# JuliaRobotics/KernelDensityEstimate.jl

Measured on AMD Instinct MI355X. Metric: gibbs_product_samples_per_sec, higher is better.
Workload: dtype f64

## Files before the change

kerneldensityestimate.jl_amd/csrc/gibbs_device.hpp:

```cpp
#pragma once
#include <hip/hip_runtime.h>

#include <cstdint>
#include <type_traits>

#include "circ_wrap.hpp"
#include "fastexp.hpp"
#include "kdehip_internal.hpp"
#include "philox.hpp"


namespace kdehip {


__device__ __forceinline__ double fast_rcp(double x) {
  double r = __builtin_amdgcn_rcp(x);
  double e = fma(-x, r, 1.0);
  r = fma(r, e, r);
  e = fma(-x, r, 1.0);
  return fma(r, e, r);
}
__device__ __forceinline__ float fast_rcp(float x) {
  float r = __builtin_amdgcn_rcpf(x);
  return fmaf(r, fmaf(-x, r, 1.0f), r);
// ... 765 lines not shown
template <int WAVES>
__device__ __forceinline__ void stage_tile(const unsigned char *__restrict__ src, unsigned char *dst,
                                           int bytes, int wave, int lane) {
  const __amdgpu_buffer_rsrc_t rsrc =
      __builtin_amdgcn_make_buffer_rsrc(const_cast<unsigned char *>(src), 0, bytes, 0x00020000);
  const int pieces = bytes >> 10;
  for (int c = wave; c < pieces; c += WAVES) {
    const int off = __builtin_amdgcn_readfirstlane(c << 10);
    __builtin_amdgcn_raw_ptr_buffer_load_lds(rsrc, (LdsVoidPtr)(dst + off), 16, lane << 4, off, 0, 0);
  }
}

template <bool BATCH>
struct LaunchView {
  const PlanDev &plan;
  const RunArgs &a;
  unsigned block;
  __device__ __forceinline__ LaunchView(const PlanDev &p, const RunArgs &a_) : plan(p), a(a_), block(blockIdx.x) {}
};
struct BatchArgs {
  int64_t Np;
  int32_t Niter, addEntropy, variant, use_tables;
  static constexpr int32_t use_screen = 0;
  uint64_t seed;
  int64_t sample_offset;
  double *points;
  int64_t *indices;
  int32_t *labels;
  static constexpr int32_t rng_philox = 1, npeers = 0, table_build = 0;
  static constexpr const double *randU = nullptr, *randN = nullptr;
  static constexpr int64_t K = 0, R = 0, nU = 0, nN = 0;
  double *peer_points[1];
  int64_t *peer_indices[1];
};
template <>
struct LaunchView<true> {
  PlanDev plan;
  BatchArgs a;
  unsigned block;
  __device__ __forceinline__ LaunchView(const PlanDev &, const RunArgs &a_) {
    const int e = ((const __attribute__((address_space(4))) int *)(a_.batch_map))[blockIdx.x];
    const auto *src = (const __attribute__((address_space(4))) kdehip_v16i *)(a_.batch + e);
    const kdehip_v16i r0 = src[0], r1 = src[1], r2 = src[2];
    BatchPlanHead h;
    BatchRun be;
    BatchFlags fl;
    __builtin_memcpy(&h, &r0, sizeof(h));
    __builtin_memcpy(&be, &r1, sizeof(be));
    __builtin_memcpy(&fl, &r2, sizeof(fl));
    plan.data = h.data; plan.perm = h.perm; plan.levels = h.levels; plan.tables = h.tables; plan.tabdesc = h.tabdesc;
    plan.tab_rows_total = h.tab_rows_total;
    plan.M = h.M; plan.L = h.L; plan.D = h.D; plan.Lt = h.Lt;
    plan.screened = 0;
    plan.circ_bits = fl.circ_bits;
    a.Np = be.Np; a.Niter = fl.Niter; a.addEntropy = fl.addEntropy; a.use_tables = fl.use_tables;
    a.variant = a_.variant;
    a.seed = be.seed; a.sample_offset = be.sample_offset;
    a.points = be.points; a.indices = be.indices; a.labels = be.labels;
    a.peer_points[0] = nullptr; a.peer_indices[0] = nullptr;
    block = blockIdx.x - static_cast<unsigned>(fl.first_block);
  }
};


}
```

kerneldensityestimate.jl_amd/csrc/gibbs_lean.hip:

```cpp
#define KDEHIP_EXP256 1
#ifndef KDEHIP_PRELOAD_MAXB
#define KDEHIP_PRELOAD_MAXB 8
#endif
#include "gibbs_device.hpp"
#include "screen_device.hpp"

namespace kdehip {

template <int I> using IC = std::integral_constant<int, I>;
template <int N, int I = 0, typename F>
__device__ __forceinline__ void static_for(F &&f) {
  if constexpr (I < N) {
    f(IC<I>{});
    static_for<N, I + 1>(f);
  }
}

#if defined(KDEHIP_LEAN_HI) || (defined(KDEHIP_LEAN_DEV_M) && KDEHIP_LEAN_DEV_M > 4)
constexpr int kLeanMinDens = 8, kLeanMaxDens = 8;
#else
constexpr int kLeanMinDens = 2, kLeanMaxDens = 4;
#endif
constexpr int kLeanMaxNormals = 128;

__device__ __forceinline__ int scalar_copy(int x) {
  int y;
  asm("s_mov_b32 %0, %1" : "=s"(y) : "s"(x));
  return y;
}

template <int D>
struct LeanTile {
  int n;
  int flags;
  int lds_off;
  int stage_bytes;
  int chunk_rows;
  int seg;
  int hdr_lo, hdr_hi;
  int B, F, last_lane;
  int uniform_bw;
  __device__ __forceinline__ int64_t hdr_off() const {
    return (static_cast<int64_t>(hdr_hi) << 32) | static_cast<uint32_t>(hdr_lo);
  }
  __device__ __forceinline__ void load(const kdehip_v8i &d) {
    n = scalar_copy(d[0]);
    flags = scalar_copy(d[1]);
    lds_off = scalar_copy(d[2]);
    stage_bytes = scalar_copy(d[3]);
    chunk_rows = scalar_copy(d[4]);
    seg = scalar_copy(d[5]);
    hdr_lo = scalar_copy(d[6]);
    hdr_hi = scalar_copy(d[7]);
    B = (n + 63) >> 6;
    last_lane = flags & 0xFF;
    uniform_bw = flags >> 8;
    F = uniform_bw ? D + 1 : 2 * D + 1;
  }
};

template <typename P, typename T, bool OK> constexpr bool kCanPreloadImpl = OK && kIsLdsPtr<P> && sizeof(T) == 8;

template <typename T, int D, int M, int WAVES, bool BATCH = false, bool SCHUNK = false>
__global__ __launch_bounds__(WAVES * 64) void gibbs_lean_kernel(PlanDev plan_, RunArgs a_) {
  const LaunchView<BATCH> view(plan_, a_);
  const PlanDev &plan = view.plan;
  const auto &a = view.a;
  constexpr bool kPrefetchRows = (WAVES <= 12) || sizeof(T) == 4 || D <= 4;
  using RowPtr = std::conditional_t<(WAVES == 16 && sizeof(T) == 8), LdsPtrSplit<T>, LdsPtr<T>>;
  constexpr int kCopyWaves = WAVES > 4 ? 4 : WAVES;
  constexpr bool kKeptRows = (WAVES <= 8);
  constexpr bool kScreen = sizeof(T) == 8 && !BATCH;
  constexpr bool kPreloadBuild = kKeptRows && kPrefetchRows;
  constexpr int kNormOff = 2048;
  constexpr int kUnifOff = kNormOff + WAVES * kLeanMaxNormals * 8;
  constexpr int kPoolOff = kUnifOff + WAVES * 1024;
  constexpr bool kCoop = kScreen && SCHUNK && WAVES == 8;
  constexpr int kXchgOff = kPoolOff + kLdsPoolBytes;
  constexpr int kXchgSlotDoubles = 32 + 4 * 64;
  constexpr int kXchgBytes = kCoop ? 64 + WAVES * kXchgSlotDoubles * 8 : 0;
  static_assert(kPoolOff + kLdsPoolBytes + kXchgBytes <= 160 * 1024, "LDS budget of one CU exceeded");
  __shared__ __attribute__((aligned(1024))) unsigned char smem[kPoolOff + kLdsPoolBytes + kXchgBytes];

  double *sExpTab = reinterpret_cast<double *>(smem);
  if (threadIdx.x < 256) sExpTab[threadIdx.x] = kExp2Tab256[threadIdx.x];
  if constexpr (kCoop) {
    if (threadIdx.x < 16) reinterpret_cast<int *>(smem + kXchgOff)[threadIdx.x] = 0;
  }

  const int lane = threadIdx.x & 63;
  const int wave = __builtin_amdgcn_readfirstlane(static_cast<int>(threadIdx.x >> 6));
  KDEHIP_PRIO_CHAIN();
  const int chain = wave;
  int64_t s = static_cast<int64_t>(view.block) * WAVES + chain;
  const bool live = s < a.Np;
  if (!live) s = a.Np - 1;
  const uint64_t gs = static_cast<uint64_t>(a.sample_offset + s);
  const void *fb = live ? static_cast<const void *>(plan.levels) : nullptr;

  const int L = plan.L;
  const T *__restrict__ data = static_cast<const T *>(plan.data);
  const LevelTable levels{(const __attribute__((address_space(4))) kdehip_v16i *)(plan.levels)};
  const StepTable steps{(const __attribute__((address_space(4))) kdehip_v8i *)(plan.levels + 2 * plan.M * (plan.L + 1))};
  unsigned char *pool = smem + kPoolOff;
  const int dl = lane < D ? lane : D - 1;
  const int vlev = a.variant % 1000;

  double *sNorm = reinterpret_cast<double *>(smem + kNormOff) + chain * kLeanMaxNormals;
  const int R = D * (L + 1);
  if (a.rng_philox) {
    for (int b = lane; 2 * b < R; b += 64) {
      double n0, n1;
      philox_normal_pair(a.seed, gs, static_cast<uint32_t>(b), n0, n1);
      sNorm[2 * b] = n0;
      if (2 * b + 1 < R) sNorm[2 * b + 1] = n1;
    }
  } else {
    for (int r = lane; r < R; r += 64) sNorm[r] = a.randN[s * a.R + r];
  }
  __syncthreads();

  T lam[M], lmu[M];
  int psel[M];

  auto adopt = [&](auto jc, const auto &ds, auto hdr, int pos) {
    constexpr int j = decltype(jc)::value;
    using TA = TileAddr<T>;
    auto e = hdr + kTileHeader + TA::row(pos >> 6, TA::stride(ds.F)) + (pos & 63) * TA::kLane;
    const T mu = e[dl * TA::kField];
    const T var = ds.uniform_bw ? hdr[dl] : e[(D + dl) * TA::kField];
    const T l = fast_rcp(var);
    lam[j] = l;
    lmu[j] = mu * l;
    psel[j] = pos;
  };
  auto product = [&](auto skipc, T &mean, T &cov) {
    constexpr int skip = decltype(skipc)::value;
    T ls = T(0), ms = T(0);
    static_for<M>([&](auto kc) {
      constexpr int k = decltype(kc)::value;
      if constexpr (k != skip) { ls += lam[k]; ms += lmu[k]; }
    });
    cov = fast_rcp(ls);
    mean = cov * ms;
  };

  auto draw = [&](const auto &ds, auto hdr, T mean, T cov, auto &&run) -> int {
    if (ds.uniform_bw) {
      EvalUniform<T, D> ev;
      ev.tab = sExpTab;
      const T c = hdr[dl] + cov;
      T cen, nin;
      EvalUniform<T, D>::operands(mean, c, true, cen, nin);
      T Pr = T(1);
#pragma unroll
      for (int d = 0; d < D; ++d) {
        ev.center[d] = lane_read(cen, d);
        ev.ninv[d] = lane_read(nin, d);
        Pr *= lane_read(c, d);
      }
      ev.scale = Num<T>::rsqrt(Pr);
      return run(ev);
    }
    EvalFast<T, D, false> ev;
    ev.tab = sExpTab;
    ev.act = 0;
#pragma unroll
    for (int d = 0; d < D; ++d) {
      ev.center[d] = lane_read(mean, d);
      ev.cov[d] = lane_read(cov, d);
    }
    return run(ev);
  };

  uint32_t c = static_cast<uint32_t>(M);
  uint32_t ubatch = 0xFFFFFFFFu;
  double *sUnif = reinterpret_cast<double *>(smem + kUnifOff) + wave * 128;
  auto next_uniform = [&]() -> double {
    const uint32_t b = c >> 7;
    if (b != ubatch) {
      ubatch = b;
      double u_even, u_odd;
      if (a.rng_philox) {
        const Philox4 r = philox_block(a.seed, gs, b * 64u + static_cast<uint32_t>(lane), 0u);
        u_even = bits_to_unit(r.v[0], r.v[1]);
        u_odd = bits_to_unit(r.v[2], r.v[3]);
      } else {
        const int64_t i0 = s * a.K + static_cast<int64_t>(b) * 128 + 2 * lane - 1;
        u_even = (i0 >= 0 && i0 < a.nU) ? a.randU[i0] : 0.5;
        u_odd = (i0 + 1 < a.nU) ? a.randU[i0 + 1] : 0.5;
      }
      wave_sync();
      sUnif[2 * lane] = u_even;
      sUnif[2 * lane + 1] = u_odd;
      wave_sync();
    }
    const double u = sUnif[c & 127u];
    ++c;
    return u;
  };

  static_for<M>([&](auto jc) {
    const LevelDesc ds = levels[decltype(jc)::value * (L + 1)];
    adopt(jc, ds, data + ds.hdr_off, 0);
  });

  const TabTable tabs{(const __attribute__((address_space(4))) kdehip_v8i *)(plan.tabdesc)};
  const T *tables = static_cast<const T *>(plan.tables);
  const int Lt = (vlev == 1 || vlev == 4 || !a.use_tables) ? 0 : plan.Lt;

  auto draw_rows = [&](const auto &ds, auto rows, const auto &ev, double u) -> int {
    using P = decltype(rows);
    return draw_label<T, P, kPrefetchRows, kKeptRows>(rows, ds, lane, ev, u, fb);
  };

  auto draw_rows_repeat = [&](const auto &ds, const T *rows, const auto &ev, double u) -> int {
    using Ev = std::decay_t<decltype(ev)>;
    if constexpr (kScreen && SCHUNK && sizeof(typename Ev::Row) <= 7 * sizeof(T) && WAVES <= 8) {
      LaneAcc<T> acc;
      KDEHIP_PRIO_ROWS();
      lane_rows_all_deep<T, Ev>(rows, ds.B, TileAddr<T>::stride(ds.F), lane, ev, acc);
      KDEHIP_PRIO_CHAIN();
      return select_or_raise<T, const T *>(acc.total(), rows, ds, lane, ev, u, fb);
    }
    return draw_rows(ds, rows, ev, u);
  };

#ifdef KDEHIP_SCREEN_STAMPS
  unsigned long long rstamp[8] = {0, 0, 0, 0, 0, 0, 0, 0}, r_prev_end = 0;
  bool rstamp_on = false;
#define RSTAMP(var) const unsigned long long var = __builtin_amdgcn_s_memtime()
#define RSTAMP_ADD(slot, t0, t1) do { if (rstamp_on) rstamp[slot] += (t1) - (t0); } while (0)
#else
#define RSTAMP(var) do {} while (0)
#define RSTAMP_ADD(slot, t0, t1) do {} while (0)
#endif
  auto step_kept = [&](auto jc, const auto &ds, auto hdr, const auto &row, T mean, T cov, double u) {
    RSTAMP(tr1);
    auto rows1 = hdr + kTileHeader;
    using P1 = decltype(rows1);
    using Ev = EvalFast<T, D, false>;
    Ev ev;
    ev.tab = sExpTab;
    ev.act = 0;
#pragma unroll
    for (int d = 0; d < D; ++d) {
      ev.center[d] = lane_read(mean, d);
      ev.cov[d] = lane_read(cov, d);
    }
#ifdef KDEHIP_SCREEN_STAMPS
    asm volatile("" ::"s"(ev.center[D - 1]), "s"(ev.cov[D - 1]));
#endif
    RSTAMP(tr2);
    RSTAMP_ADD(1, tr1, tr2);
    int pos1;
    if (ds.B == 1) {
      const T S = ev(row);
      pos1 = select_or_raise<T, P1>(S, rows1, ds, lane, ev, u, fb);
    } else if (ds.B <= 4) {
      pos1 = draw_label_kept<T, P1, Ev, 4>(rows1, ds, lane, ev, u, fb, row);
    } else {
// ... 212 lines not shown
          ev.scale = __builtin_amdgcn_rsqf(pr);
          pos = screen_draw<D, true>(rows32, ds.n, ds.B, ds.F, lane, ev, u SSTAMP_ARGS);
        } else {
          ScreenEval<D, false> ev;
          ev.a2 = a2; ev.nsum = (ds.B + 1) >> 1; ev.scale = 1.0f;
#pragma unroll
          for (int d = 0; d < D; ++d) {
            ev.cen[d] = lane_read(cen, d);
            ev.b[d] = lane_read(covf, d);
          }
          pos = screen_draw<D, false>(rows32, ds.n, ds.B, ds.F, lane, ev, u SSTAMP_ARGS);
        }
        pos = __builtin_amdgcn_readfirstlane(pos);
      }
      SSTAMP(ts2);
      SSTAMP_ADD(1, ts1, ts2);
      ++n_screened;
      if (pos < 0) {
        ++n_repeated;
        pos = __builtin_amdgcn_readfirstlane(draw(ds, hdrg, mean, cov, [&](const auto &ev) {
          return draw_rows_repeat(ds, hdrg + kTileHeader, ev, u);
        }));
      }
      SSTAMP(ts3);
      SSTAMP_ADD(2, ts2, ts3);
      adopt(jc, ds, hdrg, pos);
#ifdef KDEHIP_SCREEN_STAMPS
      {
        const double sink = lam[decltype(jc)::value] + lmu[decltype(jc)::value];
        asm volatile("" ::"v"(sink));
      }
#endif
      SSTAMP(ts4);
      SSTAMP_ADD(3, ts3, ts4);
    }
  };

  int gchunk = 0;
  auto stage_chunk = [&](const auto &ds, int r0, int half) {
    using TA = TileAddr<T>;
    const int RS = TA::stride(ds.F), rc = ds.chunk_rows;
    const int nrows = (ds.B - r0 < rc) ? (ds.B - r0) : rc;
    const int bytes = (static_cast<int>(TA::span(nrows, RS)) * int(sizeof(T)) + 1023) & ~1023;
    const unsigned char *src = reinterpret_cast<const unsigned char *>(data + ds.hdr_off() + kTileHeader + TA::row(r0, RS));
    if (wave < kCopyWaves) stage_tile<kCopyWaves>(src, pool + half * (kLdsPoolBytes / 2), bytes, wave, lane);
  };

  auto stage_schunk = [&](const LevelDesc &sc, int p0, int half) {
    using TA = TileAddr<float>;
    const int RS = TA::stride(sc.F), cp = sc.chunk_rows >> 1, npairs = (sc.B + 1) >> 1;
    const int np = (npairs - p0 < cp) ? (npairs - p0) : cp;
    const int head = p0 == 0 ? kScreenHeaderFloats : 0;
    const int bytes = ((head + np * RS) * 4 + 1023) & ~1023;
    const unsigned char *src = reinterpret_cast<const unsigned char *>(reinterpret_cast<const float *>(plan.data) + sc.hdr_off +
                                                                       (p0 == 0 ? 0 : kScreenHeaderFloats + p0 * RS));
    if (wave < kCopyWaves) stage_tile<kCopyWaves>(src, pool + half * (kLdsPoolBytes / 2), bytes, wave, lane);
  };
  auto step_screen_chunked = [&](auto jc, const auto &ds, const auto &dsp, const LevelDesc &sc, const LevelDesc &scn, bool more,
                                 bool first, bool level_start, T x) {
    if constexpr (kScreen && SCHUNK) {
      using TA = TileAddr<float>;
      T mean = x, cov = T(0);
      const bool was_pend = kCoop && pend;
      if (!first && !was_pend) product(jc, mean, cov);
      const double u = next_uniform();
      const int RS = TA::stride(sc.F), cp = sc.chunk_rows >> 1, npairs = (sc.B + 1) >> 1;
      staging_barrier();
      if (cp < npairs) stage_schunk(sc, cp, (gchunk + 1) & 1);
      else if (more) stage_schunk(scn, 0, (gchunk + 1) & 1);
      if constexpr (kCoop) {
        constexpr int j = decltype(jc)::value;
        if (!level_start) coop_resolve(IC<(j + M - 1) % M>{}, dsp, (cstep + 1) & 1);
        if (was_pend && !first) product(jc, mean, cov);
      }
      const LdsPtr<float> h32 = (LdsPtr<float>)(pool + (gchunk & 1) * (kLdsPoolBytes / 2));
      const LdsPtr<double> h64 = (LdsPtr<double>)(pool + (gchunk & 1) * (kLdsPoolBytes / 2));
      const double mu0 = h64[dl], cmin = h64[8 + dl];
      const float mmax = h32[32 + dl], valid = h32[40];
      const float *grows = reinterpret_cast<const float *>(plan.data) + sc.hdr_off + kScreenHeaderFloats;
      const int pos = __builtin_amdgcn_readfirstlane(screen_eval(ds, mu0, cmin, mmax, valid, mean, cov, [&](const auto &ev, bool ok) {
        using Ev = std::decay_t<decltype(ev)>;
        ScreenSums q;
        KDEHIP_PRIO_ROWS();
        if (ok) screen_rows<D, Ev::kUni>(h32 + kScreenHeaderFloats + lane * TA::kLane, npairs < cp ? npairs : cp, RS, ev, q);
        ++gchunk;
        for (int p0 = cp; p0 < npairs; p0 += cp, ++gchunk) {
          staging_barrier();
          if (p0 + cp < npairs) stage_schunk(sc, p0 + cp, (gchunk + 1) & 1);
          else if (more) stage_schunk(scn, 0, (gchunk + 1) & 1);
          const int np = (npairs - p0 < cp) ? (npairs - p0) : cp;
          if (ok) screen_rows<D, Ev::kUni>((LdsPtr<float>)(pool + (gchunk & 1) * (kLdsPoolBytes / 2)) + lane * TA::kLane, np, RS, ev, q);
        }
        KDEHIP_PRIO_CHAIN();
        if (!ok) return -1;
        return screen_decide<D, Ev::kUni, true>(grows, ds.n, ds.B, RS, lane, ev, u, q.values(), q.moments() SSTAMP_ARGS);
      }));
      if constexpr (kCoop) {
        ++n_screened;
        if (pos < 0) {
          ++n_repeated;
          coop_post(mean, cov, u);
        } else {
          adopt(jc, ds, data + ds.hdr_off(), pos);
        }
        ++cstep;
      } else {
        screen_finish(jc, ds, pos, mean, cov, u);
      }
    }
  };

#ifdef KDEHIP_EXPERIMENTS
  const int Lrun = (vlev >= 100 && vlev - 100 < L) ? vlev - 100 : L;
#else
  const int Lrun = L;
#endif
  for (int l = 1; l <= Lrun; ++l) {
    T x;
    {
      T mean, cov;
      product(IC<-1>{}, mean, cov);
      x = mean + Num<T>::sqrt(cov) * static_cast<T>(sNorm[(l - 1) * D + dl]);
    }
    const int level_mode = scalar_copy(levels[l].stage_mode);
    auto tile_raw = [&](int j) -> kdehip_v8i { return steps.raw(j * (L + 1) + l); };
    auto tile = [&](int j) -> LeanTile<D> {
      LeanTile<D> t;
      t.load(tile_raw(j));
      return t;
    };
    const int mode = vlev == 1 ? int(kStageGlobal) : level_mode;
    const bool tabulated = (l <= Lt);
    const int npass = tabulated ? 1 : a.Niter + 1;

    bool screened = false, screen_streamed = false, screen_chunked = false;
    if constexpr (kScreen) {
      if (a.use_screen && vlev != 1) {
        const int smode = scalar_copy(levels[M * (L + 1) + l].stage_mode);
        screened = smode == kStageScreen;
        screen_streamed = smode == kStageScreenStream;
        if constexpr (SCHUNK) screen_chunked = smode == kStageScreenChunked;
      }
    }
#ifdef KDEHIP_SCREEN_STAMPS
    rstamp_on = (vlev >= 300 && l == vlev - 300) && view.block == 3 && wave == 5;
    r_prev_end = 0;
#endif
    if (screened) {
#ifdef KDEHIP_SCREEN_STAMPS
      sstamp_on = (l == ((vlev >= 200) ? vlev - 200 : L)) && view.block == 3 && wave == 5;
#endif
      auto screen = [&](int j) -> LevelDesc { return levels[(M + j) * (L + 1) + l]; };
      staging_barrier();
      static_for<M>([&](auto jc) {
        const LevelDesc sc = screen(decltype(jc)::value);
        stage_tile<WAVES>(reinterpret_cast<const unsigned char *>(reinterpret_cast<const float *>(plan.data) + sc.hdr_off),
                          pool + sc.lds_off, sc.stage_bytes, wave, lane);
      });
      staging_barrier();
      for (int p = 0; p < npass; ++p)
        static_for<M>([&](auto jc) {
          const LeanTile<D> ds = tile(decltype(jc)::value);
          step_screen(jc, ds, ds.lds_off, p == 0, x);
        });
    } else if (screen_streamed) {
      auto screen = [&](int j) -> LevelDesc { return levels[(M + j) * (L + 1) + l]; };
      auto stage_screen = [&](const LevelDesc &sc, int half, auto wc) {
        constexpr int W = decltype(wc)::value;
        if (wave < W)
          stage_tile<W>(reinterpret_cast<const unsigned char *>(reinterpret_cast<const float *>(plan.data) + sc.hdr_off),
                        pool + half * (kLdsPoolBytes / 2), sc.stage_bytes, wave, lane);
      };
      staging_barrier();
      stage_screen(screen(0), 0, IC<WAVES>{});
      int t = 0;
      const int nsteps = npass * M;
      for (int p = 0; p < npass; ++p)
        static_for<M>([&](auto jc) {
          constexpr int j = decltype(jc)::value;
          constexpr int jn = (j + 1 == M) ? 0 : j + 1;
          const LeanTile<D> ds = tile(j);
          const LevelDesc scn = screen(jn);
          staging_barrier();
          constexpr bool kLateCopy = kCopyWaves < WAVES;
          if (!kLateCopy && t + 1 < nsteps) stage_screen(scn, (t + 1) & 1, IC<WAVES>{});
          step_screen(jc, ds, (t & 1) * (kLdsPoolBytes / 2), p == 0, x);
          if (kLateCopy && t + 1 < nsteps) stage_screen(scn, (t + 1) & 1, IC<kCopyWaves>{});
          ++t;
        });
    } else if (screen_chunked) {
      auto screen = [&](int j) -> LevelDesc { return levels[(M + j) * (L + 1) + l]; };
      staging_barrier();
      stage_schunk(screen(0), 0, gchunk & 1);
      int t = 0;
      const int nsteps = npass * M;
      for (int p = 0; p < npass; ++p)
        static_for<M>([&](auto jc) {
          constexpr int j = decltype(jc)::value;
          constexpr int jn = (j + 1 == M) ? 0 : j + 1;
          constexpr int jp = (j + M - 1) % M;
          const LeanTile<D> ds = tile(j);
          step_screen_chunked(jc, ds, tile(jp), screen(j), screen(jn), t + 1 < nsteps, p == 0, t == 0, x);
          ++t;
        });
      if constexpr (kCoop) {
        __syncthreads();
        coop_resolve(IC<M - 1>{}, tile(M - 1), (cstep + 1) & 1);
      }
    } else if (mode == kStageResident) {
      staging_barrier();
      static_for<M>([&](auto jc) {
        const LeanTile<D> ds = tile(decltype(jc)::value);
        stage_tile<WAVES>(reinterpret_cast<const unsigned char *>(data + ds.hdr_off()), pool + ds.lds_off, ds.stage_bytes, wave, lane);
      });
      staging_barrier();
      for (int p = 0; p < npass; ++p)
        static_for<M>([&](auto jc) {
          const LeanTile<D> ds = tile(decltype(jc)::value);
          step(jc, ds, (RowPtr)(pool + ds.lds_off), p == 0, x);
        });
    } else if (mode == kStageStream) {
      staging_barrier();
      {
// ... 72 lines not shown
          adopt(jc, ds, hdr, pos);
          ++t;
        });
    } else {
      for (int p = 0; p < npass; ++p)
        static_for<M>([&](auto jc) {
          const LeanTile<D> ds = tile(decltype(jc)::value);
          step(jc, ds, data + ds.hdr_off(), p == 0, x);
        });
    }

    if (tabulated) {
      TabDesc td[M];
      static_for<M>([&](auto jc) { td[decltype(jc)::value] = tabs[decltype(jc)::value * (L + 1) + l]; });
      uint32_t word = 0;
      static_for<M>([&](auto jc) { word |= static_cast<uint32_t>(psel[decltype(jc)::value]) << td[decltype(jc)::value].shift; });
      word = __builtin_amdgcn_readfirstlane(word);
      for (int p = 1; p <= a.Niter; ++p)
        static_for<M>([&](auto jc) {
          constexpr int j = decltype(jc)::value;
          const TabDesc &tj = td[j];
          const uint32_t cfg = (word & ((1u << tj.shift) - 1u)) | ((word >> (tj.shift + tj.bits)) << tj.shift);
          const T *row = tables + tj.off + static_cast<int64_t>(cfg) * (tj.n + 1);
          const int n = tj.n;
          const T incl = row[lane < n ? lane : n];
          const double u = next_uniform();
          const T total = lane_read(incl, n < 64 ? n : 63);
          int pos;
          if (!(total >= Num<T>::tiny_total())) {
            count_fallback(fb, lane);
            const LeanTile<D> dk = tile(j);
            const T wl = ((LdsPtr<T>)(pool + dk.lds_off) + kTileHeader)[(dk.F - 1) * TileAddr<T>::kField + (n - 1) * TileAddr<T>::kLane];
            int z = n - 1;
            if (wl > T(0)) {
              z = static_cast<int>(ceil(u * static_cast<double>(n))) - 1;
              z = z < 0 ? 0 : (z > n - 1 ? n - 1 : z);
            }
            pos = __builtin_amdgcn_readfirstlane(z);
          } else {
            const T target = static_cast<T>(u) * total;
            unsigned long long hit = __ballot(target <= incl);
            if (n < 64) hit &= (1ull << n) - 1ull;
            pos = hit ? (__ffsll(hit) - 1) : (n - 1);
          }
          word = (word & ~(((1u << tj.bits) - 1u) << tj.shift)) | (static_cast<uint32_t>(pos) << tj.shift);
        });
      static_for<M>([&](auto jc) {
        constexpr int j = decltype(jc)::value;
        const int pk = static_cast<int>((word >> td[j].shift) & ((1u << td[j].bits) - 1u));
        const LeanTile<D> dk = tile(j);
        adopt(jc, dk, (LdsPtr<T>)(pool + dk.lds_off), pk);
      });
    }
    if (a.labels && live && lane == 0) {
      static_for<M>([&](auto jc) {
        constexpr int j = decltype(jc)::value;
        a.labels[(s * M + j) * L + (l - 1)] = plan.perm[levels[j * (L + 1) + l].perm_off + psel[j]];
      });
    }
    if (l == L && live && lane == 0) {
      static_for<M>([&](auto jc) {
        constexpr int j = decltype(jc)::value;
        const int64_t label = static_cast<int64_t>(plan.perm[levels[j * (L + 1) + l].perm_off + psel[j]]) + 1;
        a.indices[s * M + j] = label;
        for (int k = 0; k < a.npeers; ++k) a.peer_indices[k][s * M + j] = label;
      });
    }
  }

#ifdef KDEHIP_SCREEN_STAMPS
  if (view.block == 3 && wave == 5 && lane == 0)
    for (int k = 0; k < 8; ++k) { g_screen_stamps[k] = sstamp[k]; g_screen_stamps[8 + k] = rstamp[k]; }
#endif
  if constexpr (kScreen) {
    if (live && lane == 0 && n_screened != 0u) {
      unsigned long long *cnt = reinterpret_cast<unsigned long long *>(const_cast<LevelDesc *>(plan.levels));
      atomicAdd(cnt - 3, static_cast<unsigned long long>(n_screened));
      if (n_repeated != 0u) atomicAdd(cnt - 2, static_cast<unsigned long long>(n_repeated));
    }
  }
  {
    T mean, cov;
    product(IC<-1>{}, mean, cov);
    T xf = mean;
    if (a.addEntropy) xf = mean + Num<T>::sqrt(cov) * static_cast<T>(sNorm[L * D + dl]);
    if (live && lane < D) {
      a.points[s * D + lane] = static_cast<double>(xf);
      for (int k = 0; k < a.npeers; ++k) a.peer_points[k][s * D + lane] = static_cast<double>(xf);
    }
  }
}


template <typename T, int D, int M, int WAVES>
static void launch_lean_waves(const PlanDev &plan, const RunArgs &args, hipStream_t stream) {
  const int64_t blocks = (args.Np + WAVES - 1) / WAVES;
  if constexpr (sizeof(T) == 8 && WAVES >= 8) {
    if (M == 8 || (plan.screened == 2 && args.use_screen)) {
      hipLaunchKernelGGL((gibbs_lean_kernel<T, D, M, WAVES, false, true>), dim3(static_cast<unsigned>(blocks)), dim3(WAVES * 64),
                         0, stream, plan, args);
      return;
    }
  }
  if constexpr (!(sizeof(T) == 8 && WAVES >= 8 && M == 8))
    hipLaunchKernelGGL((gibbs_lean_kernel<T, D, M, WAVES>), dim3(static_cast<unsigned>(blocks)), dim3(WAVES * 64), 0,
                       stream, plan, args);
}

static int set_geometry(const PlanDev &, RunArgs &args, int) { return lean_waves(args.Np, args.variant); }

template <typename T, int D, int M>
static int launch_lean_m(const PlanDev &plan, const RunArgs &args_in, hipStream_t stream) {
  RunArgs args = args_in;
  const int waves = set_geometry(plan, args, sizeof(T) == 8 ? 64 : 32);
  if (waves == 16) launch_lean_waves<T, D, M, 16>(plan, args, stream);
  else if (waves == 8) launch_lean_waves<T, D, M, 8>(plan, args, stream);
  else launch_lean_waves<T, D, M, 4>(plan, args, stream);
  const hipError_t e = hipGetLastError();
  if (e != hipSuccess)
    return set_error(KDEHIP_ERR_HIP, std::string("kernel launch failed: ") + hipGetErrorString(e));
  return KDEHIP_OK;
}

#ifndef KDEHIP_DIM
#error "compile gibbs_lean.hip with -DKDEHIP_DIM=<1..8>"
#endif
#define KDEHIP_CAT2(a, b) a##b
#define KDEHIP_CAT(a, b) KDEHIP_CAT2(a, b)

template <typename T, int D, int M>
static int launch_lean_m_hi(const PlanDev &plan, const RunArgs &args_in, hipStream_t stream) {
  RunArgs args = args_in;
  const int waves = set_geometry(plan, args, sizeof(T) == 8 ? 64 : 32);
  if (waves == 16) launch_lean_waves<T, D, M, 16>(plan, args, stream);
  else if (waves == 8) launch_lean_waves<T, D, M, 8>(plan, args, stream);
  else return kLeanNotCovered;
  const hipError_t e = hipGetLastError();
  if (e != hipSuccess)
    return set_error(KDEHIP_ERR_HIP, std::string("kernel launch failed: ") + hipGetErrorString(e));
  return KDEHIP_OK;
}

#if !defined(KDEHIP_LEAN_HI) && !defined(KDEHIP_LEAN_F32) && !defined(KDEHIP_LEAN_DEV)
template <int D, int M>
static void launch_lean_batch_m(const PlanDev &plan, const RunArgs &args, hipStream_t stream) {
  constexpr int W = 16;
  hipLaunchKernelGGL((gibbs_lean_kernel<double, D, M, W, true>), dim3(static_cast<unsigned>(args.Np / W)), dim3(W * 64), 0,
                     stream, plan, args);
}
int KDEHIP_CAT(launch_lean_batch_d, KDEHIP_DIM)(int M, const PlanDev &plan, const RunArgs &args, void *stream) {
  constexpr int D = KDEHIP_DIM;
  hipStream_t st = static_cast<hipStream_t>(stream);
  if (args.Np <= 0) return KDEHIP_OK;
  switch (M) {
    case 2: launch_lean_batch_m<D, 2>(plan, args, st); break;
    case 3: launch_lean_batch_m<D, 3>(plan, args, st); break;
    case 4: launch_lean_batch_m<D, 4>(plan, args, st); break;
    default: return set_error(KDEHIP_ERR_UNSUPPORTED, "batched launch: 2..4 densities");
  }
// ... 75 lines not shown
```

kerneldensityestimate.jl_amd/csrc/kdehip_internal.hpp:

```cpp
#pragma once

#include <hip/hip_runtime_api.h>

#include <cstddef>
#include <cstdint>
#include <functional>
#include <string>
#include <vector>

#include "../../include/kdehip.h"

namespace kdehip {

int set_error(int code, const std::string &msg);
const char *last_error_cstr();

constexpr int kTileHeader = 8;
#if defined(__HIPCC__)
#define KDEHIP_TILE_HD __host__ __device__ inline
#else
#define KDEHIP_TILE_HD inline
#endif
template <int ELEM_BYTES>
struct TileAddrBytes {
// ... 35 lines not shown
  int32_t last_lane;
  int32_t chunk_rows;
  int32_t seg;
};
constexpr int kMaxSegDesc = 8;
inline int32_t seg_geometry(int B, int rc) {
  if (rc <= 0 || rc > 64) return 0;
  const int cps = 64 / rc, sr = cps * rc, nseg = (B + sr - 1) / sr;
  return nseg <= kMaxSegDesc ? (cps | (nseg << 16)) : 0;
}
static_assert(sizeof(LevelDesc) == 64, "LevelDesc is read with scalar loads; keep it 64 bytes");

struct StepDesc {
  int32_t n;
  int32_t flags;
  int32_t lds_off;
  int32_t stage_bytes;
  int32_t chunk_rows;
  int32_t seg;
  int32_t hdr_lo, hdr_hi;
};
static_assert(sizeof(StepDesc) == 32, "StepDesc is read with one 32-byte scalar load");

constexpr int kScreenHeaderFloats = 48;
constexpr int kScreenMaxRows = 64;
constexpr int kScreenMaxRowsChunked = 128;
constexpr float kScreenMaxAbsMean = 65536.0f;
constexpr double kScreenMinVar = 1.0 / 128.0, kScreenMaxVar = 256.0;
constexpr float kScreenMaxNa = 0x1p-11f;
constexpr float kScreenMaxA2 = 1.14e7f;

struct TabDesc {
  int64_t off;
  int64_t row_base;
  int32_t n;
  int32_t ncfg;
  int32_t shift;
  int32_t bits;
};
static_assert(sizeof(TabDesc) == 32, "TabDesc is read with one 32-byte scalar load");
constexpr int64_t kTabMaxEntries = 512 * 1024;
constexpr int64_t kTabMinChains = 16;

struct PlanDev {
  const void *data;
  const int32_t *perm;
  const LevelDesc *levels;
  const void *tables;
  const TabDesc *tabdesc;
  int64_t tab_rows_total;
  int32_t M, L, D, Lt;
  int32_t screened;
  uint32_t circ_bits;
  int32_t reserved_[2];
};

constexpr int kMaxPeers = 7;
struct BatchEntry;
struct RunArgs {
  int64_t Np;
  int32_t Niter;
  int32_t addEntropy;
  int32_t rng_philox;
  int32_t variant;
  int32_t table_build;
  int32_t use_tables;
  int32_t use_screen;
  const double *randU;
  const double *randN;
  int64_t K, R;
  int64_t nU, nN;
  uint64_t seed;
  int64_t sample_offset;
  double *points;
  int64_t *indices;
  int32_t *labels;
  int32_t npeers;
  double *peer_points[kMaxPeers];
  int64_t *peer_indices[kMaxPeers];
  const BatchEntry *batch;
  const int32_t *batch_map;
};

struct BatchPlanHead {
  const void *data;
  const int32_t *perm;
  const LevelDesc *levels;
  const void *tables;
  const TabDesc *tabdesc;
  int64_t tab_rows_total;
  int32_t M, L, D, Lt;
};
struct BatchRun {
  int32_t reserved_[4];
  int64_t Np;
  uint64_t seed;
  int64_t sample_offset;
  double *points;
  int64_t *indices;
  int32_t *labels;
};
struct BatchFlags {
  int32_t Niter, addEntropy, use_tables;
  int32_t first_block;
  uint32_t circ_bits;
  int32_t pad_[11];
};
// ... 85 lines not shown
```

kerneldensityestimate.jl_amd/csrc/product.hip:

```cpp
#include <hip/hip_runtime.h>

#include <atomic>
#include <cstdlib>
#include <chrono>
#include <cstdio>
#include <cstdlib>
#include <cstring>
#include <mutex>
#include <new>
#include <string>
#include <vector>

#include "call_block.hpp"
#include "device_density.hpp"
#include "entry_helpers.hpp"
#include "manifold_arg.hpp"
#include "kdehip_internal.hpp"
#include "phase_timer.hpp"

namespace kdehip { extern std::atomic<unsigned> g_peer_epoch; }
#include "philox.hpp"

using namespace kdehip;

// ... 216 lines not shown
    im.off_count = im.off_lev - sizeof(unsigned long long);
    im.off_tab = align256(im.off_lev + level_table_bytes(im.host));
    im.off_perm = align256(im.off_tab + ntab * sizeof(TabDesc));
    im.off_data = align256(im.off_perm + nperm * sizeof(int32_t));
    im.off_tables = align256(im.off_data + nelem * esz);
    im.total = im.off_tables + static_cast<size_t>(im.host.tab_entries) * esz;
    int ndev = 0;
    if (hipGetDeviceCount(&ndev) != hipSuccess || ndev <= 0)
      return set_error(KDEHIP_ERR_NO_DEVICE, "no HIP device available (libkdehip has no CPU fallback by design)");
    KDEHIP_CHECK(cached_host_malloc(&im.h_blob, im.off_tables));
    im.blob_bytes = im.off_tables;
    const double us_alloc = us();
    unsigned char *hb = static_cast<unsigned char *>(im.h_blob);
    std::memset(hb, 0, im.off_lev);
    copy_level_table(im.host, hb + im.off_lev);
    std::memcpy(hb + im.off_tab, im.host.tabdesc.data(), ntab * sizeof(TabDesc));
    const bool ok = pack_fill(im.host, trees, hb + im.off_data, reinterpret_cast<int32_t *>(hb + im.off_perm));
    if (timing)
      std::fprintf(stderr, "kdehip image%s: layout %.0f us | pinned block %.0f us | tiles filled %.0f us\n",
                   ok ? "" : " (fast form refused: again in the generic form)", us_layout, us_alloc, us());
    if (ok) break;
    cached_host_free(im.h_blob, im.blob_bytes);
    im.h_blob = nullptr;
  }
  std::vector<int32_t>().swap(im.host.front);
  return KDEHIP_OK;
}

void bind_plan(kdehip_product *p, size_t off_lev, size_t off_count, size_t off_tab, size_t off_perm, size_t off_data,
               size_t off_tables, size_t total) {
  unsigned char *base = static_cast<unsigned char *>(p->d_blob);
  p->d_levels = reinterpret_cast<LevelDesc *>(base + off_lev);
  p->d_tabdesc = reinterpret_cast<TabDesc *>(base + off_tab);
  p->d_perm = reinterpret_cast<int32_t *>(base + off_perm);
  p->d_data = base + off_data;
  p->d_fallbacks = reinterpret_cast<unsigned long long *>(base + off_count);
  p->d_tables = p->host.tab_entries ? base + off_tables : nullptr;
  p->packed_bytes = static_cast<int64_t>(total);
  p->dev.data = p->d_data;
  p->dev.perm = p->d_perm;
  p->dev.levels = p->d_levels;
  p->dev.tables = p->d_tables;
  p->dev.tabdesc = p->d_tabdesc;
  p->dev.tab_rows_total = p->host.tab_rows;
  p->dev.M = p->host.M;
  p->dev.L = p->host.L;
  p->dev.D = p->host.D;
  p->dev.Lt = (p->mode == kModeGeneric || p->mode == kModeFastCirc) ? 0 : p->host.Lt;
  p->dev.circ_bits = p->circ_bits;
  p->dev.screened = (p->mode == kModeFast && !p->host.screens.empty()) ? 1 : 0;
  if (p->dev.screened)
    for (const LevelDesc &sc : p->host.screens)
      if (sc.stage_mode == kStageScreenChunked) p->dev.screened = 2;
}

int instantiate(const PlanImage &im, int device, kdehip_product **out, bool wait = true, uint32_t circ_bits = 0) {
  *out = nullptr;
  kdehip_product *p = new (std::nothrow) kdehip_product();
  if (!p) return set_error(KDEHIP_ERR_ALLOC, "out of host memory");
  DeviceGuard guard;
  int rc = guard.enter(device);
  if (rc != KDEHIP_OK) { delete p; return rc; }
  p->device = device;
  p->precision = im.precision;
  p->host = im.host;
  p->fast = p->host.fast;
  p->mode = !p->host.fast ? kModeGeneric : (p->host.all_active ? kModeFast : kModeFastMasked);
  p->circ_bits = circ_bits;
  if (circ_bits != 0u && p->host.fast) p->mode = kModeFastCirc;
  hipError_t e = cached_malloc(&p->d_blob, im.total);
  if (e == hipSuccess) p->blob_bytes = im.total;
  if (e == hipSuccess) e = hipMemcpyAsync(p->d_blob, im.h_blob, im.off_tables, hipMemcpyHostToDevice, call_stream());
  if (e == hipSuccess && wait) e = hipStreamSynchronize(call_stream());
  if (e != hipSuccess) {
    const std::string m = std::string("plan upload: ") + hipGetErrorString(e);
    kdehip_product_destroy(p);
    return set_error(KDEHIP_ERR_HIP, m);
  }
  bind_plan(p, im.off_lev, im.off_count, im.off_tab, im.off_perm, im.off_data, im.off_tables, im.total);
  *out = p;
  return KDEHIP_OK;
}

inline bool alias_devices() {
  static const bool on = [] { const char *e = std::getenv("KDEHIP_ALIAS_DEVICES"); return e && e[0] == '1'; }();
  return on;
}
inline int phys(int d) {
  if (!alias_devices()) return d;
  int n = 1;
  if (hipGetDeviceCount(&n) != hipSuccess || n <= 0) n = 1;
  return d % n;
}

inline int64_t share_begin(int64_t Np, int g, int G) { return Np * g / G; }

int check_devices(int device, int ngpus) {
  if (ngpus < 1) return set_error(KDEHIP_ERR_ARG, "ngpus must be >= 1");
  int n = 0;
  if (hipGetDeviceCount(&n) != hipSuccess || n <= 0)
    return set_error(KDEHIP_ERR_NO_DEVICE, "no HIP device available (libkdehip has no CPU fallback by design)");
  if (alias_devices() ? (device < 0 || ngpus > KDEHIP_MAX_DENS) : (device < 0 || device + ngpus > n))
    return set_error(KDEHIP_ERR_ARG, "device range outside the visible devices");
  return KDEHIP_OK;
}

// ... 1111 lines not shown
```

Measured before the change: 4.360 million.

## Add resident-only lean kernel twin and keep cold args in kernarg

Adds a compile-time twin of the lean Gibbs kernel that assumes every level is LDS-resident. When the host-side plan shows all tiles are resident, this twin is launched and the staged/streamed code paths are compiled out. Rarely used run arguments (randN, randU, labels, output pointers) are now re-read from the kernarg segment at the point of use, and hot base pointers are pinned to scalar registers. Both changes aim to lower register pressure and code size in the hot loop, at the cost of an extra kernel instantiation and more host logic for picking the variant.

```diff
diff --git a/kerneldensityestimate.jl_amd/csrc/gibbs_device.hpp b/kerneldensityestimate.jl_amd/csrc/gibbs_device.hpp
--- a/kerneldensityestimate.jl_amd/csrc/gibbs_device.hpp
+++ b/kerneldensityestimate.jl_amd/csrc/gibbs_device.hpp
@@ -841,6 +841,7 @@
     plan.tab_rows_total = h.tab_rows_total;
     plan.M = h.M; plan.L = h.L; plan.D = h.D; plan.Lt = h.Lt;
     plan.screened = 0;
+    plan.resident = 0;
     plan.circ_bits = fl.circ_bits;
     a.Np = be.Np; a.Niter = fl.Niter; a.addEntropy = fl.addEntropy; a.use_tables = fl.use_tables;
     a.variant = a_.variant;
diff --git a/kerneldensityestimate.jl_amd/csrc/gibbs_lean.hip b/kerneldensityestimate.jl_amd/csrc/gibbs_lean.hip
--- a/kerneldensityestimate.jl_amd/csrc/gibbs_lean.hip
+++ b/kerneldensityestimate.jl_amd/csrc/gibbs_lean.hip
@@ -27,6 +27,14 @@
   int y;
   asm("s_mov_b32 %0, %1" : "=s"(y) : "s"(x));
   return y;
+}
+
+template <typename P>
+__device__ __forceinline__ P *scalar_copy(P *p) {
+  const uint64_t v = reinterpret_cast<uint64_t>(p);
+  const uint32_t lo = static_cast<uint32_t>(scalar_copy(static_cast<int>(v)));
+  const uint32_t hi = static_cast<uint32_t>(scalar_copy(static_cast<int>(v >> 32)));
+  return reinterpret_cast<P *>((static_cast<uint64_t>(hi) << 32) | lo);
 }
 
 template <int D>
@@ -61,8 +69,16 @@
 
 template <typename P, typename T, bool OK> constexpr bool kCanPreloadImpl = OK && kIsLdsPtr<P> && sizeof(T) == 8;
 
-template <typename T, int D, int M, int WAVES, bool BATCH = false, bool SCHUNK = false>
+template <typename T> struct Staged {};
+template <typename TT> struct LeanPrec { using type = TT; static constexpr bool kStaged = false; };
+template <typename T> struct LeanPrec<Staged<T>> { using type = T; static constexpr bool kStaged = true; };
+template <typename T, int WAVES, bool BATCH, bool SCHUNK>
+constexpr bool kLeanHasTwin = sizeof(T) == 8 && WAVES >= 8 && !BATCH && !SCHUNK;
+
+template <typename TT, int D, int M, int WAVES, bool BATCH = false, bool SCHUNK = false>
 __global__ __launch_bounds__(WAVES * 64) void gibbs_lean_kernel(PlanDev plan_, RunArgs a_) {
+  using T = typename LeanPrec<TT>::type;
+  constexpr bool STAGED = LeanPrec<TT>::kStaged || !kLeanHasTwin<T, WAVES, BATCH, SCHUNK>;
   const LaunchView<BATCH> view(plan_, a_);
   const PlanDev &plan = view.plan;
   const auto &a = view.a;
@@ -72,6 +88,8 @@
   constexpr bool kKeptRows = (WAVES <= 8);
   constexpr bool kScreen = sizeof(T) == 8 && !BATCH;
   constexpr bool kPreloadBuild = kKeptRows && kPrefetchRows;
+  constexpr bool kResidentOnly = !STAGED;
+  static_assert(STAGED || !SCHUNK, "chunked screen tiles are staged tiles");
   constexpr int kNormOff = 2048;
   constexpr int kUnifOff = kNormOff + WAVES * kLeanMaxNormals * 8;
   constexpr int kPoolOff = kUnifOff + WAVES * 1024;
@@ -96,12 +114,25 @@
   const bool live = s < a.Np;
   if (!live) s = a.Np - 1;
   const uint64_t gs = static_cast<uint64_t>(a.sample_offset + s);
-  const void *fb = live ? static_cast<const void *>(plan.levels) : nullptr;
-
+  const T *__restrict__ data = scalar_copy(static_cast<const T *>(plan.data));
+  const LevelDesc *const plan_levels = scalar_copy(plan.levels);
+  const int32_t *const plan_perm = scalar_copy(plan.perm);
+  const void *fb = live ? static_cast<const void *>(plan_levels) : nullptr;
+
+  auto cold = [&]() -> decltype(auto) {
+    if constexpr (BATCH) {
+      return (view.a);
+    } else {
+      constexpr size_t kOff = (sizeof(PlanDev) + alignof(RunArgs) - 1) / alignof(RunArgs) * alignof(RunArgs);
+      auto p = (const __attribute__((address_space(4))) RunArgs *)((const __attribute__((address_space(4))) char *)
+                                                                        __builtin_amdgcn_kernarg_segment_ptr() + kOff);
+      asm volatile("" : "+s"(p));
+      return (*p);
+    }
+  };
   const int L = plan.L;
-  const T *__restrict__ data = static_cast<const T *>(plan.data);
-  const LevelTable levels{(const __attribute__((address_space(4))) kdehip_v16i *)(plan.levels)};
-  const StepTable steps{(const __attribute__((address_space(4))) kdehip_v8i *)(plan.levels + 2 * plan.M * (plan.L + 1))};
+  const LevelTable levels{(const __attribute__((address_space(4))) kdehip_v16i *)(plan_levels)};
+  const StepTable steps{(const __attribute__((address_space(4))) kdehip_v8i *)(plan_levels + 2 * plan.M * (plan.L + 1))};
   unsigned char *pool = smem + kPoolOff;
   const int dl = lane < D ? lane : D - 1;
   const int vlev = a.variant % 1000;
@@ -116,7 +147,7 @@
       if (2 * b + 1 < R) sNorm[2 * b + 1] = n1;
     }
   } else {
-    for (int r = lane; r < R; r += 64) sNorm[r] = a.randN[s * a.R + r];
+    for (int r = lane; r < R; r += 64) { const auto &ca = cold(); sNorm[r] = ca.randN[s * ca.R + r]; }
   }
   __syncthreads();
 
@@ -182,13 +213,14 @@
       ubatch = b;
       double u_even, u_odd;
       if (a.rng_philox) {
-        const Philox4 r = philox_block(a.seed, gs, b * 64u + static_cast<uint32_t>(lane), 0u);
+        const Philox4 r = philox_block(cold().seed, gs, b * 64u + static_cast<uint32_t>(lane), 0u);
         u_even = bits_to_unit(r.v[0], r.v[1]);
         u_odd = bits_to_unit(r.v[2], r.v[3]);
       } else {
-        const int64_t i0 = s * a.K + static_cast<int64_t>(b) * 128 + 2 * lane - 1;
-        u_even = (i0 >= 0 && i0 < a.nU) ? a.randU[i0] : 0.5;
-        u_odd = (i0 + 1 < a.nU) ? a.randU[i0 + 1] : 0.5;
+        const auto &ca = cold();
+        const int64_t i0 = s * ca.K + static_cast<int64_t>(b) * 128 + 2 * lane - 1;
+        u_even = (i0 >= 0 && i0 < ca.nU) ? ca.randU[i0] : 0.5;
+        u_odd = (i0 + 1 < ca.nU) ? ca.randU[i0 + 1] : 0.5;
       }
       wave_sync();
       sUnif[2 * lane] = u_even;
@@ -206,7 +238,7 @@
   });
 
   const TabTable tabs{(const __attribute__((address_space(4))) kdehip_v8i *)(plan.tabdesc)};
-  const T *tables = static_cast<const T *>(plan.tables);
+  const T *tables = scalar_copy(static_cast<const T *>(plan.tables));
   const int Lt = (vlev == 1 || vlev == 4 || !a.use_tables) ? 0 : plan.Lt;
 
   auto draw_rows = [&](const auto &ds, auto rows, const auto &ev, double u) -> int {
@@ -525,7 +557,7 @@
     const int np = (npairs - p0 < cp) ? (npairs - p0) : cp;
     const int head = p0 == 0 ? kScreenHeaderFloats : 0;
     const int bytes = ((head + np * RS) * 4 + 1023) & ~1023;
-    const unsigned char *src = reinterpret_cast<const unsigned char *>(reinterpret_cast<const float *>(plan.data) + sc.hdr_off +
+    const unsigned char *src = reinterpret_cast<const unsigned char *>(reinterpret_cast<const float *>(data) + sc.hdr_off +
                                                                        (p0 == 0 ? 0 : kScreenHeaderFloats + p0 * RS));
     if (wave < kCopyWaves) stage_tile<kCopyWaves>(src, pool + half * (kLdsPoolBytes / 2), bytes, wave, lane);
   };
@@ -550,7 +582,7 @@
       const LdsPtr<double> h64 = (LdsPtr<double>)(pool + (gchunk & 1) * (kLdsPoolBytes / 2));
       const double mu0 = h64[dl], cmin = h64[8 + dl];
       const float mmax = h32[32 + dl], valid = h32[40];
-      const float *grows = reinterpret_cast<const float *>(plan.data) + sc.hdr_off + kScreenHeaderFloats;
+      const float *grows = reinterpret_cast<const float *>(data) + sc.hdr_off + kScreenHeaderFloats;
       const int pos = __builtin_amdgcn_readfirstlane(screen_eval(ds, mu0, cmin, mmax, valid, mean, cov, [&](const auto &ev, bool ok) {
         using Ev = std::decay_t<decltype(ev)>;
         ScreenSums q;
@@ -602,7 +634,7 @@
       t.load(tile_raw(j));
       return t;
     };
-    const int mode = vlev == 1 ? int(kStageGlobal) : level_mode;
+    const int mode = kResidentOnly ? int(kStageResident) : vlev == 1 ? int(kStageGlobal) : level_mode;
     const bool tabulated = (l <= Lt);
     const int npass = tabulated ? 1 : a.Niter + 1;
 
@@ -611,7 +643,7 @@
       if (a.use_screen && vlev != 1) {
         const int smode = scalar_copy(levels[M * (L + 1) + l].stage_mode);
         screened = smode == kStageScreen;
-        screen_streamed = smode == kStageScreenStream;
+        screen_streamed = !kResidentOnly && smode == kStageScreenStream;
         if constexpr (SCHUNK) screen_chunked = smode == kStageScreenChunked;
       }
     }
@@ -627,7 +659,7 @@
       staging_barrier();
       static_for<M>([&](auto jc) {
         const LevelDesc sc = screen(decltype(jc)::value);
-        stage_tile<WAVES>(reinterpret_cast<const unsigned char *>(reinterpret_cast<const float *>(plan.data) + sc.hdr_off),
+        stage_tile<WAVES>(reinterpret_cast<const unsigned char *>(reinterpret_cast<const float *>(data) + sc.hdr_off),
                           pool + sc.lds_off, sc.stage_bytes, wave, lane);
       });
       staging_barrier();
@@ -641,7 +673,7 @@
       auto stage_screen = [&](const LevelDesc &sc, int half, auto wc) {
         constexpr int W = decltype(wc)::value;
         if (wave < W)
-          stage_tile<W>(reinterpret_cast<const unsigned char *>(reinterpret_cast<const float *>(plan.data) + sc.hdr_off),
+          stage_tile<W>(reinterpret_cast<const unsigned char *>(reinterpret_cast<const float *>(data) + sc.hdr_off),
                         pool + half * (kLdsPoolBytes / 2), sc.stage_bytes, wave, lane);
       };
       staging_barrier();
@@ -820,18 +852,19 @@
         adopt(jc, dk, (LdsPtr<T>)(pool + dk.lds_off), pk);
       });
     }
-    if (a.labels && live && lane == 0) {
+    if (int32_t *const labels = cold().labels; labels && live && lane == 0) {
       static_for<M>([&](auto jc) {
         constexpr int j = decltype(jc)::value;
-        a.labels[(s * M + j) * L + (l - 1)] = plan.perm[levels[j * (L + 1) + l].perm_off + psel[j]];
+        labels[(s * M + j) * L + (l - 1)] = plan_perm[levels[j * (L + 1) + l].perm_off + psel[j]];
       });
     }
     if (l == L && live && lane == 0) {
+      const auto &ca = cold();
       static_for<M>([&](auto jc) {
         constexpr int j = decltype(jc)::value;
-        const int64_t label = static_cast<int64_t>(plan.perm[levels[j * (L + 1) + l].perm_off + psel[j]]) + 1;
-        a.indices[s * M + j] = label;
-        for (int k = 0; k < a.npeers; ++k) a.peer_indices[k][s * M + j] = label;
+        const int64_t label = static_cast<int64_t>(plan_perm[levels[j * (L + 1) + l].perm_off + psel[j]]) + 1;
+        ca.indices[s * M + j] = label;
+        for (int k = 0; k < ca.npeers; ++k) ca.peer_indices[k][s * M + j] = label;
       });
     }
   }
@@ -842,7 +875,7 @@
 #endif
   if constexpr (kScreen) {
     if (live && lane == 0 && n_screened != 0u) {
-      unsigned long long *cnt = reinterpret_cast<unsigned long long *>(const_cast<LevelDesc *>(plan.levels));
+      unsigned long long *cnt = reinterpret_cast<unsigned long long *>(const_cast<LevelDesc *>(plan_levels));
       atomicAdd(cnt - 3, static_cast<unsigned long long>(n_screened));
       if (n_repeated != 0u) atomicAdd(cnt - 2, static_cast<unsigned long long>(n_repeated));
     }
@@ -850,11 +883,12 @@
   {
     T mean, cov;
     product(IC<-1>{}, mean, cov);
+    const auto &ca = cold();
     T xf = mean;
-    if (a.addEntropy) xf = mean + Num<T>::sqrt(cov) * static_cast<T>(sNorm[L * D + dl]);
+    if (ca.addEntropy) xf = mean + Num<T>::sqrt(cov) * static_cast<T>(sNorm[L * D + dl]);
     if (live && lane < D) {
-      a.points[s * D + lane] = static_cast<double>(xf);
-      for (int k = 0; k < a.npeers; ++k) a.peer_points[k][s * D + lane] = static_cast<double>(xf);
+      ca.points[s * D + lane] = static_cast<double>(xf);
+      for (int k = 0; k < ca.npeers; ++k) ca.peer_points[k][s * D + lane] = static_cast<double>(xf);
     }
   }
 }
@@ -870,9 +904,18 @@
       return;
     }
   }
-  if constexpr (!(sizeof(T) == 8 && WAVES >= 8 && M == 8))
+  if constexpr (!(sizeof(T) == 8 && WAVES >= 8 && M == 8)) {
+    if constexpr (kLeanHasTwin<T, WAVES, false, false>) {
+      const bool resident = plan.resident == 1 || (plan.resident == 2 && args.use_screen);
+      if (!resident || args.variant % 1000 == 1) {
+        hipLaunchKernelGGL((gibbs_lean_kernel<Staged<T>, D, M, WAVES>), dim3(static_cast<unsigned>(blocks)), dim3(WAVES * 64), 0,
+                           stream, plan, args);
+        return;
+      }
+    }
     hipLaunchKernelGGL((gibbs_lean_kernel<T, D, M, WAVES>), dim3(static_cast<unsigned>(blocks)), dim3(WAVES * 64), 0,
                        stream, plan, args);
+  }
 }
 
 static int set_geometry(const PlanDev &, RunArgs &args, int) { return lean_waves(args.Np, args.variant); }
diff --git a/kerneldensityestimate.jl_amd/csrc/kdehip_internal.hpp b/kerneldensityestimate.jl_amd/csrc/kdehip_internal.hpp
--- a/kerneldensityestimate.jl_amd/csrc/kdehip_internal.hpp
+++ b/kerneldensityestimate.jl_amd/csrc/kdehip_internal.hpp
@@ -111,7 +111,8 @@
   int32_t M, L, D, Lt;
   int32_t screened;
   uint32_t circ_bits;
-  int32_t reserved_[2];
+  int32_t resident;
+  int32_t reserved_;
 };
 
 constexpr int kMaxPeers = 7;
diff --git a/kerneldensityestimate.jl_amd/csrc/product.hip b/kerneldensityestimate.jl_amd/csrc/product.hip
--- a/kerneldensityestimate.jl_amd/csrc/product.hip
+++ b/kerneldensityestimate.jl_amd/csrc/product.hip
@@ -292,6 +292,13 @@
   if (p->dev.screened)
     for (const LevelDesc &sc : p->host.screens)
       if (sc.stage_mode == kStageScreenChunked) p->dev.screened = 2;
+  int resident = 1;
+  for (size_t i = 0; i < p->host.levels.size(); ++i) {
+    if (i % static_cast<size_t>(p->host.L + 1) == 0 || p->host.levels[i].stage_mode == kStageResident) continue;
+    const bool screen_resident = p->dev.screened && p->host.screens[i].stage_mode == kStageScreen;
+    resident = (resident && screen_resident) ? 2 : 0;
+  }
+  p->dev.resident = p->mode == kModeFast ? resident : 0;
 }
 
 int instantiate(const PlanImage &im, int device, kdehip_product **out, bool wait = true, uint32_t circ_bits = 0) {
```

New measurement: 4.430 million (median of 6 runs). 1.6% higher.
